# microsoft/Cream

Hardware: AMD Instinct MI355X
Metric: images/sec (whole node) AutoFormer-S supernet step @224^2 (higher is better)
Workload: dtype bf16; 1 GPU; AutoFormer-S supernet train step, random-path sampling (random.seed(epoch)), per-GPU batch 128, 224x224, AdamW, grad all-reduce RCCL; global_batch=128, parallelism=dp1, wgrad_partials=bf16 split-K partial tiles (within 1.9e-3 of fp32 partials), mixup=on-device, in the timed region

## Files before the change

### cream_amd/_lib.py

```python
import ctypes
import os

_HERE = os.path.dirname(os.path.abspath(__file__))
LIB_PATH = os.path.join(_HERE, "libcream_amd.so")

CREAM_OK = 0
_ERRORS = {
    -1: "CREAM_ERR_BAD_ARG (null pointer, negative size or unsupported stride)",
    -2: "CREAM_ERR_BAD_DTYPE (element type not supported by this entry point)",
    -3: "CREAM_ERR_LAUNCH (HIP kernel launch failed)",
    -4: "CREAM_ERR_TOO_LARGE (shape exceeds what the kernel family supports)",
}

F32, F16, BF16, F64 = 0, 1, 2, 3


class CreamLibraryError(RuntimeError):
    pass


_c = ctypes
_vp, _i, _i64, _f = _c.c_void_p, _c.c_int, _c.c_int64, _c.c_float

SIGNATURES = {
# ... 53 lines not shown
    "cream_block_wgrad_bf16": (_i, [_i]),
    "cream_colsum128_slabs": (_i, [_i]),
    "cream_colsum128": (_i, [_vp, _vp, _i, _i, _vp]),
    "cream_gelu_bwd_colsum": (_i, [_vp, _vp, _vp, _vp, _i, _i, _vp]),
    "cream_scale_cast_colsum": (_i, [_vp, _vp, _vp, _vp, _i, _i, _i, _vp]),
    "cream_grad_finalize": (_i, [_vp, _i, _vp]),
    "cream_gemm_rows_per_colsum_slab": (_i, []),
    "cream_gemm_nt256": (_i, [_i]),
    "cream_gemm_nt8": (_i, [_i]),
    "cream_linear_fwd": (_i, [_vp, _vp, _vp, _vp, _i, _i, _i, _i64, _vp]),
    "cream_linear_fwd_seg": (_i, [_vp, _vp, _vp, _vp, _i, _i, _i, _i64, _i, _i64, _vp]),
    "cream_linear_gelu_fwd": (_i, [_vp, _vp, _vp, _vp, _vp, _i, _i, _i, _i64, _vp]),
    "cream_linear_gelu_fwd_pad": (_i, [_vp, _vp, _vp, _vp, _vp, _i, _i, _i, _i, _i64, _vp]),
    "cream_linear_dgrad": (_i, [_vp, _vp, _vp, _i, _i, _i, _i64, _vp]),
    "cream_linear_dgrad_seg": (_i, [_vp, _vp, _vp, _i, _i, _i, _i64, _i, _i64, _vp]),
    "cream_linear_dgrad_mul": (_i, [_vp, _vp, _vp, _vp, _vp, _i, _i, _i, _i64, _vp]),
    "cream_linear_wgrad_splits": (_i, [_i, _i, _i]),
    "cream_linear_wgrad_splits_bf16": (_i, [_i, _i, _i]),
    "cream_gemm_tn8": (_i, [_i]),
    "cream_gemm_nthalf": (_i, [_i]),
    "cream_gemm_ntopt": (_i, [_i]),
    "cream_gemm_stagger": (_i, [_i]),
    "cream_block_layout_epoch": (_i, []),
    "cream_cu_reserve": (_i, [_i]),
    "cream_mixup_cutmix": (_i, [_vp, _vp, _vp, _i, _i, _i, _i, _i, _f, _i, _i, _i, _i, _i, _f, _vp]),
    "cream_image_batch_plan": (_i64, [_vp, _i, _i, _i]),
    "cream_image_batch_transform": (_i, [_vp, _vp, _i64, _vp, _vp, _i, _i, _i, _vp, _vp, _vp, _i64, _vp]),
    "cream_cu_count": (_i, []),
    "cream_linear_wgrad_parts": (_i, [_vp, _vp, _vp, _vp, _i, _i, _i, _i, _vp]),
    "cream_linear_wgrad_parts_bf16": (_i, [_vp, _vp, _vp, _vp, _i, _i, _i, _i, _vp]),
    "cream_param_job_tiles": (_i, [_i, _i]),
    "cream_adamw_step": (_i, [_vp, _vp, _i, _i, _i, _c.c_double, _c.c_double, _c.c_double, _c.c_double, _i64, _vp]),
    "cream_soft_ce": (_i, [_vp, _vp, _vp, _vp, _i, _i, _i, _f, _vp]),
    "cream_linear_f32_fwd": (_i, [_vp, _vp, _vp, _vp, _i, _i, _i, _i64, _i64, _i, _i, _vp]),
    "cream_bmm_f32": (_i, [_vp, _vp, _vp, _i, _i, _i, _vp, _vp, _vp, _i, _i, _vp]),
    "cream_linear_f32_dgrad": (_i, [_vp, _vp, _vp, _i, _i, _i, _i64, _i, _i, _vp]),
    "cream_linear_f32_wgrad": (_i, [_vp, _vp, _vp, _vp, _i, _i, _i, _i64, _i64, _i, _i, _vp]),
    "cream_ln_f32_fwd": (_i, [_vp, _vp, _vp, _vp, _vp, _vp, _i, _i, _f, _vp]),
    "cream_ln_f32_bwd": (_i, [_vp, _vp, _vp, _vp, _vp, _vp, _vp, _i, _i, _vp]),
    "cream_block_prof_enable": (_i, [_i]),
    "cream_block_prof_kinds": (_i, []),
    "cream_block_prof_name": (_c.c_char_p, [_i]),
    "cream_block_prof_collect": (_i, [_vp, _vp, _vp, _vp]),
    "cream_slices_copy": (_i, [_vp, _i, _vp, _i, _i, _vp]),
    "cream_block_fwd_workspace": (_i64, [_vp, _vp, _vp, _vp]),
    "cream_block_fwd": (_i, [_vp, _vp, _vp, _vp, _vp, _vp, _vp]),
    "cream_block_bwd_workspace": (_i64, [_vp, _vp, _vp, _vp]),
    "cream_block_bwd": (_i, [_vp, _vp, _vp, _vp, _vp, _vp, _vp, _vp, _i, _i64, _vp, _vp, _i, _vp, _vp]),
    "cream_image_augment_workspace": (_i64, [_i, _i, _i, _i]),
    "cream_image_augment_u8": (_i, [_vp, _vp, _i, _i, _i, _vp, _vp, _i, _vp, _i64, _vp]),
    "cream_image_batch_plan_aug": (_i64, [_vp, _i, _i, _i, _vp, _i]),
    "cream_image_batch_transform_aug": (_i, [_vp, _vp, _i64, _vp, _vp, _i, _i, _i, _vp, _vp, _vp, _vp, _i, _vp, _i64, _vp]),
}

MAX_GRAD_JOBS = 24


class GradJob(ctypes.Structure):
    _fields_ = [("dst", _vp), ("src", _vp), ("ld", _i64), ("pstride", _i64),
                ("nparts", _c.c_int32), ("rows", _c.c_int32), ("cols", _c.c_int32),
                ("interleave", _c.c_int32), ("src_bf16", _c.c_int32), ("overwrite", _c.c_int32)]

class ImageDesc(ctypes.Structure):
    _fields_ = ([("offset", _i64)] +
                [(n, _c.c_int32) for n in ("height", "width", "row_stride", "box_top", "box_left", "box_h", "box_w", "resized_h",
                                           "resized_w", "win_top", "win_left", "flip", "row0", "nrows")] +
# ... 91 lines not shown
```

### cream_amd/autoformer/block.py

```python
import ctypes
import os

import torch

from .. import _lib, timing
from . import fused_attention

def _p(t):
    return ctypes.c_void_p(t.data_ptr()) if t is not None else ctypes.c_void_p(0)


def _stream():
    return ctypes.c_void_p(torch.cuda.current_stream().cuda_stream)


def ln_fwd(x2d, gamma, beta, eps):
    M, E = x2d.shape
    y = torch.empty((M, E), dtype=torch.bfloat16, device=x2d.device)
    mean = torch.empty(M, dtype=torch.float32, device=x2d.device)
    rstd = torch.empty(M, dtype=torch.float32, device=x2d.device)
    with timing.region("ln_fwd", nbytes=M * E * 6):
        _lib.check(_lib.load().cream_ln_fwd(_p(y), _p(mean), _p(rstd), _p(x2d), _p(gamma), _p(beta), M, E,
                                           float(eps), _stream()), "cream_ln_fwd")
    return y, mean, rstd
# ... 47 lines not shown
    out = torch.empty_like(x2d)
    with timing.region("residual_add", nbytes=x2d.numel() * 10):
        _lib.check(_lib.load().cream_residual_add(_p(out), _p(x2d), _p(y), _p(sample_scale), x2d.numel(), per_sample,
                                                  _stream()), "cream_residual_add")
    return out


def scale_cast(x2d, sample_scale, per_sample):
    out = torch.empty(x2d.shape, dtype=torch.bfloat16, device=x2d.device)
    with timing.region("scale_cast", nbytes=x2d.numel() * 6):
        _lib.check(_lib.load().cream_scale_cast(_p(out), _p(x2d), _p(sample_scale), x2d.numel(), per_sample,
                                                _stream()), "cream_scale_cast")
    return out


def colsum(a):
    M, C = a.shape
    lib = _lib.load()
    partial = torch.empty((lib.cream_colsum_slabs(M), C), dtype=torch.float32, device=a.device)
    with timing.region("colsum", nbytes=a.numel() * 2):
        _lib.check(lib.cream_colsum(_p(partial), _p(a), M, C, _stream()), "cream_colsum")
    return partial.sum(dim=0)


def gelu_bwd_colsum(dg, h):
    M, C = h.shape
    lib = _lib.load()
    dh = torch.empty_like(h)
    partial = torch.empty((lib.cream_colsum128_slabs(M), C), dtype=torch.float32, device=h.device)
    with timing.region("gelu_bwd", nbytes=h.numel() * 6):
        _lib.check(lib.cream_gelu_bwd_colsum(_p(dh), _p(partial), _p(dg), _p(h), M, C, _stream()),
                   "cream_gelu_bwd_colsum")
    return dh, partial


def scale_cast_colsum(x2d, sample_scale, rows_per_sample):
    M, C = x2d.shape
    lib = _lib.load()
    out = torch.empty((M, C), dtype=torch.bfloat16, device=x2d.device)
    partial = torch.empty((lib.cream_colsum128_slabs(M), C), dtype=torch.float32, device=x2d.device)
    with timing.region("scale_cast", nbytes=x2d.numel() * 6):
        _lib.check(lib.cream_scale_cast_colsum(_p(out), _p(partial), _p(x2d), _p(sample_scale), rows_per_sample,
                                               M, C, _stream()), "cream_scale_cast_colsum")
    return out, partial


def colsum128(a):
    M, C = a.shape
    lib = _lib.load()
    partial = torch.empty((lib.cream_colsum128_slabs(M), C), dtype=torch.float32, device=a.device)
    with timing.region("colsum", nbytes=a.numel() * 2):
        _lib.check(lib.cream_colsum128(_p(partial), _p(a), M, C, _stream()), "cream_colsum128")
    return partial


def linear_fwd(x, w, bias, N, K, out=None):
    M = x.shape[0]
    if out is None:
        out = torch.empty((M, N), dtype=torch.bfloat16, device=x.device)
    with timing.region("gemm_nt", flops=2 * M * N * K):
        _lib.check(_lib.load().cream_linear_fwd(_p(out), _p(x), _p(w), _p(bias), M, N, K, w.stride(0), _stream()),
                   "cream_linear_fwd")
    return out


def linear_fwd_seg(x, w3, bias, N, K, nseg, out=None):
# ... 480 lines not shown


def head(head_mod, feat):
    return HeadFunction.apply(feat, head_mod.weight, head_mod.bias, head_mod)


class SoftTargetCEFunction(torch.autograd.Function):

    @staticmethod
    def forward(ctx, logits, target):
        lib = _lib.load()
        B, C = logits.shape
        x = logits.contiguous()
        t = target.contiguous()
        rows = torch.empty(B, dtype=torch.float32, device=x.device)
        dl = torch.empty((B, C), dtype=torch.float32, device=x.device)
        code = _lib.BF16 if x.dtype == torch.bfloat16 else _lib.F32
        _lib.check(lib.cream_soft_ce(_p(rows), _p(dl), _p(x), _p(t), B, C, code, 1.0 / B, _stream()), "cream_soft_ce")
        ctx.save_for_backward(dl)
        ctx.out_dtype = logits.dtype
        return rows.mean()

    @staticmethod
    def backward(ctx, g):
        (dl,) = ctx.saved_tensors
        out = torch.empty(dl.shape, dtype=ctx.out_dtype, device=dl.device)
        torch.mul(dl, g, out=out)
        return out, None


def soft_ce_supported(logits, target):
    return (logits.is_cuda and logits.dim() == 2 and logits.shape[1] <= 2048 and logits.dtype in (torch.bfloat16, torch.float32)
            and target.dtype == torch.float32 and target.shape == logits.shape and not target.requires_grad)


class PatchEmbedFunction(torch.autograd.Function):

    @staticmethod
    def forward(ctx, patches, weight, bias, pe, E):
        ops = patch_operands(pe)
        K = ops.w.shape[1]
        y = linear_fwd(patches, ops.w, ops.b, E, K)
        ctx.save_for_backward(patches)
        ctx.pe, ctx.E, ctx.K = pe, E, K
        return y

    @staticmethod
    def backward(ctx, dy):
        (patches,) = ctx.saved_tensors
        pe, E, K = ctx.pe, ctx.E, ctx.K
        dy = dy.to(torch.bfloat16).contiguous()
        parts, bparts = linear_wgrad_parts(dy, patches, want_bias=True)
        w = pe.proj.weight
        gw = parts.sum(0).view(E, *w.shape[1:])
        gb = bparts.sum(0)
        return None, _pad_rows(gw, w.shape[0]), _pad_rows(gb, w.shape[0]), None, None


def _pad_rows(g, rows):
    if g.shape[0] == rows:
        return g
    out = g.new_zeros((rows,) + tuple(g.shape[1:]))
    out[:g.shape[0]] = g
    return out


# ... 302 lines not shown
    ent = blk.__dict__.get(_GRADS_KEY)
    if ent is not None and all(p.grad is g for p, g in ent[1]):
        return ent[0]
    params = _block_params(blk) + (ln1.weight, ln1.bias, ln2.weight, ln2.bias) + _tables(at)
    gr = [_ensure_grad(p) for p in params]
    g = _lib.BlockGrads()
    g.wqkv, g.bqkv, g.wproj, g.bproj, g.w1, g.b1, g.w2, g.b2 = (t.data_ptr() for t in gr[:8])
    g.ld_qkv, g.ld_proj, g.ld_w1, g.ld_w2 = gr[0].stride(0), gr[2].stride(0), gr[4].stride(0), gr[6].stride(0)
    g.ln1_g, g.ln1_b, g.ln2_g, g.ln2_b = (t.data_ptr() for t in gr[8:12])
    g.tkv, g.tkh, g.tvv, g.tvh = (t.data_ptr() for t in gr[12:16])
    g.ldt = gr[12].stride(0)
    blk.__dict__[_GRADS_KEY] = (g, list(zip(params, gr)))
    return g


def _ws_layout(d):
    lib = _lib.load()
    key = (d.B, d.N, d.E, d.H, d.F, lib.cream_block_layout_epoch())
    hit = _ws_cache.get(key)
    if hit is None:
        o = [ctypes.c_int64() for _ in range(6)]
        ft = lib.cream_block_fwd_workspace(ctypes.byref(d), ctypes.byref(o[0]), ctypes.byref(o[1]), ctypes.byref(o[2]))
        bt = lib.cream_block_bwd_workspace(ctypes.byref(d), ctypes.byref(o[3]), ctypes.byref(o[4]), ctypes.byref(o[5]))
        if ft < 0 or bt < 0:
            raise RuntimeError("cream_amd: block workspace query failed")
        hit = _ws_cache[key] = (ft, o[0].value, o[1].value, o[2].value, bt, o[3].value, o[4].value, o[5].value)
    return hit


class StackFunction(torch.autograd.Function):

    @staticmethod
    def forward(ctx, x, scales, blks, *tail_args):
        tail_w, tail_b, tail_eps = (tuple(tail_args) + (None, None, 1e-5)[len(tail_args):])[:3]
        ctx.ntail = len(tail_args)
        ctx.tail = tail_w is not None
        if NATIVE_BLOCK:
            return StackFunction._forward_native(ctx, x, scales, blks, tail_w, tail_b, tail_eps)
        assert tail_w is None, "the fused tail needs the native block driver"
        B, N, E = x.shape
        M = B * N
        cur = x.contiguous().view(M, E)
        pend = None
        saved, dims = [], []
        for i, blk in enumerate(blks):
            dp1 = scales[i, 0] if scales is not None else None
            dp2 = scales[i, 1] if scales is not None else None
            x1, f, d, sv = _block_forward(blk, cur, pend, dp1, B, N)
            saved.extend(sv)
            dims.append(d)
            cur, pend = x1, (f, dp2)
        out = residual_add(cur, pend[0], pend[1], N * E)
        ctx.native = False
        ctx.blks = list(blks)
        ctx.dims = dims
        ctx.nsaved = len(saved) // len(blks)
        ctx.has_scales = scales is not None
        ctx.save_for_backward(*saved, *([scales] if scales is not None else []))
        return out.view(B, N, E)

    @staticmethod
    def _forward_native(ctx, x, scales, blks, tail_w=None, tail_b=None, tail_eps=1e-5):
        B, N, E = x.shape
        lib = _lib.load()
        x = x.contiguous()
        dev = x.device
        stream = ctypes.c_void_p(torch.cuda.current_stream(dev).cuda_stream)
        sc_ptr = scales.data_ptr() if scales is not None else 0
        cur, pend_f, pend_s = x.data_ptr(), 0, 0
        descs, wss, xptrs = [], [], []
        inference = not any(ctx.needs_input_grad)
        for i, blk in enumerate(blks):
            d = _block_desc(blk, B, N)
            d.inference = 1 if inference else 0
            ft, off_x, off_x1, off_f = _ws_layout(d)[:4]
            ws = torch.empty(ft, dtype=torch.uint8, device=dev)
            wp = ws.data_ptr()
            dp1 = sc_ptr + (2 * i) * B * 4 if sc_ptr else 0
            _lib.check(lib.cream_block_fwd(ctypes.byref(d), wp, cur, pend_f, pend_s, dp1, stream), "cream_block_fwd")
            xptrs.append(wp + off_x if pend_f else cur)
            descs.append(d)
            wss.append(ws)
            cur, pend_f, pend_s = wp + off_x1, wp + off_f, (sc_ptr + (2 * i + 1) * B * 4 if sc_ptr else 0)
        ctx.native = True
        ctx.blks = list(blks)
        ctx.descs = descs
        ctx.xptrs = xptrs
        ctx.shape = (B, N, E)
        ctx.has_scales = scales is not None
        if tail_w is not None:
            f32 = dict(dtype=torch.float32, device=dev)
            pooled, xm = torch.empty((B, E), **f32), torch.empty((B, E), **f32)
            stats = torch.empty((2, B * N), **f32)
            part = torch.empty((B, lib.cream_tail_chunks(N), E), **f32)
            gamma, beta = tail_w.detach()[:E].contiguous(), tail_b.detach()[:E].contiguous()
            _lib.check(lib.cream_tail_fwd(pooled.data_ptr(), xm.data_ptr(), part.data_ptr(), stats[0].data_ptr(),
                                          stats[1].data_ptr(), cur, pend_f, pend_s, gamma.data_ptr(), beta.data_ptr(), B, N, E,
                                          tail_eps, stream), "cream_tail_fwd")
            ctx.tail_ptrs = (cur, pend_f, pend_s)
            ctx.tail_shapes = (tuple(tail_w.shape), tuple(tail_b.shape))
            ctx.tail_params = (tail_w, tail_b) if isinstance(tail_w, torch.nn.Parameter) else None
            ctx.save_for_backward(x, *wss, *([scales] if scales is not None else []), xm, stats, gamma)
            return pooled
        out = torch.empty((B, N, E), dtype=torch.float32, device=dev)
        _lib.check(lib.cream_residual_add(out.data_ptr(), cur, pend_f, pend_s, B * N * E, N * E, stream), "cream_residual_add")
        ctx.save_for_backward(x, *wss, *([scales] if scales is not None else []))
        return out

    @staticmethod
    def backward(ctx, dout):
        if ctx.native:
            return StackFunction._backward_native(ctx, dout)
        blks = ctx.blks
        tens = ctx.saved_tensors
        scales = tens[-1] if ctx.has_scales else None
        ns = ctx.nsaved
        B, N, E = ctx.dims[0][:3]
        dx = dout.contiguous().view(B * N, E)
        L = len(blks)
        df, part = scale_cast_colsum(dx, scales[L - 1, 1] if scales is not None else None, N)
        pb2 = (part, part.shape[0], E, 0)
        for i in range(L - 1, -1, -1):
            dp1 = scales[i, 0] if scales is not None else None
            prev_scale = scales[i - 1, 1] if (scales is not None and i > 0) else None
            dx, df, pb2 = _block_backward(blks[i], ctx.dims[i], dp1, tens[i * ns:(i + 1) * ns], dx, df, pb2,
                                          prev_scale, i > 0)
        join_side_stream_at_end_of_backward(dx.device)
        return (dx.view(B, N, E), None, None) + (None, None, None)[:ctx.ntail]

    @staticmethod
    def _backward_native(ctx, dout):
        blks = ctx.blks
        tens = ctx.saved_tensors
        tail = None
        if ctx.tail:
            tens, tail = tens[:-3], tens[-3:]
        scales = tens[-1] if ctx.has_scales else None
        wss = tens[1:1 + len(blks)]
        B, N, E = ctx.shape
        M = B * N
        lib = _lib.load()
        dev = dout.device
        stream = ctypes.c_void_p(torch.cuda.current_stream(dev).cuda_stream)
        if WGRAD_SIDE_STREAM:
            side_st = _side_stream(dev)
            side = ctypes.c_void_p(side_st.cuda_stream)
        else:
            side_st, side = None, stream
        sc_ptr = scales.data_ptr() if scales is not None else 0
        L = len(blks)
        tail_grads = (None, None)
        if tail is not None:
            xm, stats, gamma = tail
            g = dout.contiguous().float()
            dx_t = torch.empty((M, E), dtype=torch.float32, device=dev)
            df_t = torch.empty((M, E), dtype=torch.bfloat16, device=dev)
            part = torch.empty((lib.cream_ln_partials(), E), dtype=torch.float32, device=dev)
            x1p, fp, sp = ctx.tail_ptrs
            _lib.check(lib.cream_tail_bwd(dx_t.data_ptr(), df_t.data_ptr(), part.data_ptr(), g.data_ptr(), x1p, fp,
                                          stats[0].data_ptr(), stats[1].data_ptr(), gamma.data_ptr(), sp, B, N, E, stream),
                       "cream_tail_bwd")
            wshape, bshape = ctx.tail_shapes
            if NATIVE_ENDS_GRADS and ctx.tail_params is not None:
                tw, tb = ctx.tail_params
                gx = g * xm
                jobs = GradJobs()
                jobs.add(tw, gx, B, E, 1, E)
                jobs.add(tb, g, B, E, 1, E)
                _accumulate_and_notify(jobs, [tw, tb])
            else:
                gw = torch.zeros(wshape, dtype=torch.float32, device=dev)
                gb = torch.zeros(bshape, dtype=torch.float32, device=dev)
                torch.sum(g * xm, dim=0, out=gw[:E])
                torch.sum(g, dim=0, out=gb[:E])
                tail_grads = (gw, gb)
        else:
            dx_t = dout.contiguous().view(M, E)
            df_t, part = scale_cast_colsum(dx_t, scales[L - 1, 1] if scales is not None else None, N)
        keep = [dx_t, df_t, part]
        dx, df, pb2, pb2_parts, pb2_stride = dx_t.data_ptr(), df_t.data_ptr(), part.data_ptr(), part.shape[0], E
        ws = None
        off_dx = 0
        for i in range(L - 1, -1, -1):
            d = ctx.descs[i]
            bt, off_dx, off_dfp, off_pl1 = _ws_layout(d)[4:]
            ws = torch.empty(bt, dtype=torch.uint8, device=dev)
            keep.append(ws)
            wp = ws.data_ptr()
            g = _block_grads(blks[i])
            dp1 = sc_ptr + (2 * i) * B * 4 if sc_ptr else 0
            prev = sc_ptr + (2 * (i - 1) + 1) * B * 4 if (sc_ptr and i > 0) else 0
            _lib.check(lib.cream_block_bwd(ctypes.byref(d), ctypes.byref(g), wss[i].data_ptr(), ctx.xptrs[i], wp, dx, df, pb2,
                                           pb2_parts, pb2_stride, dp1, prev, 1 if i > 0 else 0, stream, side),
                       "cream_block_bwd")
            if _grad_ready_hooks:
                if side_st is not None:
                    with torch.cuda.stream(side_st):
                        _notify(blks[i])
                else:
                    _notify(blks[i])
            dx, df = wp + off_dx, wp + off_dfp
            pb2, pb2_parts, pb2_stride = wp + off_pl1 + 2 * E * 4, lib.cream_ln_partials(), 3 * E
        join_side_stream_at_end_of_backward(dev, keep + [t for t in tens if t is not None and t.is_cuda])
        out = ws[off_dx:off_dx + M * E * 4].view(torch.float32).view(B, N, E)
        return (out, None, None) + (tail_grads[0], tail_grads[1], None)[:ctx.ntail]


class BlockFunction:

    @staticmethod
    def apply(x, dp1, dp2, blk):
        scales = None
        if dp1 is not None or dp2 is not None:
            ones = torch.ones(x.shape[0], device=x.device, dtype=torch.float32)
            scales = torch.stack([dp1 if dp1 is not None else ones, dp2 if dp2 is not None else ones]).unsqueeze(0)
        return StackFunction.apply(x, scales, [blk], None, None, 1e-5)
```

### cream_amd/autoformer/engine.py

```python
import random

import torch
import torch.nn.functional as F

from . import block as _block
from .supernet import Vision_TransformerSuper

SEARCH_SPACES = {
    'T': dict(embed_dim=256, depth=14, num_heads=4, mlp_ratio=4.0,
              choices=dict(mlp_ratio=[3.5, 4], num_heads=[3, 4], depth=[12, 13, 14], embed_dim=[192, 216, 240])),
    'S': dict(embed_dim=448, depth=14, num_heads=7, mlp_ratio=4.0,
              choices=dict(mlp_ratio=[3.0, 3.5, 4.0], num_heads=[5, 6, 7], depth=[12, 13, 14],
                           embed_dim=[320, 384, 448])),
    'B': dict(embed_dim=640, depth=16, num_heads=10, mlp_ratio=4.0,
              choices=dict(mlp_ratio=[3.0, 3.5, 4.0], num_heads=[8, 9, 10], depth=[14, 15, 16],
                           embed_dim=[528, 576, 624])),
}


def sample_configs(choices):
    depth = random.choice(choices['depth'])
    config = {dim: [random.choice(choices[dim]) for _ in range(depth)] for dim in ('mlp_ratio', 'num_heads')}
    config['embed_dim'] = [random.choice(choices['embed_dim'])] * depth
    config['layer_num'] = depth
    return config


def build_supernet(size='S', drop_path_rate=0.1, num_classes=1000, img_size=224, **overrides):
    s = SEARCH_SPACES[size]
    kw = dict(img_size=img_size, patch_size=16, embed_dim=s['embed_dim'], depth=s['depth'],
              num_heads=s['num_heads'], mlp_ratio=s['mlp_ratio'], qkv_bias=True, drop_rate=0.0,
              drop_path_rate=drop_path_rate, gp=True, num_classes=num_classes, max_relative_position=14,
              relative_position=True, change_qkv=True, abs_pos=True)
    kw.update(overrides)
    return Vision_TransformerSuper(**kw)


def soft_target_cross_entropy(logits, target):
    if logits.is_cuda and _block.soft_ce_supported(logits, target):
        return _block.SoftTargetCEFunction.apply(logits, target)
    return torch.sum(-target * F.log_softmax(logits.float(), dim=-1), dim=-1).mean()


def param_groups(model, weight_decay=0.05):
    skip = model.no_weight_decay() if hasattr(model, 'no_weight_decay') else set()
    decay, no_decay = [], []
    for name, p in model.named_parameters():
        if not p.requires_grad:
            continue
        (no_decay if (p.dim() <= 1 or name.endswith('.bias') or name in skip) else decay).append(p)
    return [{'params': no_decay, 'weight_decay': 0.0}, {'params': decay, 'weight_decay': weight_decay}]


class NativeAdamW(torch.optim.Optimizer):

    def __init__(self, model, param_groups, lr, betas=(0.9, 0.999), eps=1e-8):
        super().__init__(param_groups, dict(lr=lr, betas=betas, eps=eps, weight_decay=0.0))
        self.model = model
        self._cream_rewrites_operands = True
        self._steps = 0
        self._table = None
        self._grads = ()
        self._plist = ()
        self._ops = []
        for g in self.param_groups:
            for p in g['params']:
                self.state[p] = dict(exp_avg=torch.zeros_like(p, memory_format=torch.contiguous_format),
                                     exp_avg_sq=torch.zeros_like(p, memory_format=torch.contiguous_format))

    def _build(self):
        wd = {p: g['weight_decay'] for g in self.param_groups for p in g['params']}
        for p in wd:
            st = self.state[p]
            for k in ('exp_avg', 'exp_avg_sq'):
# ... 78 lines not shown
    return torch.optim.AdamW(groups, lr=scaled, betas=(0.9, 0.999), eps=1e-8)


class SupernetTrainer:

    def __init__(self, model, optimizer, choices, reducer=None, amp_dtype=torch.bfloat16, max_norm=0.0, mixup_fn=None):
        self.mixup_fn = mixup_fn
        self.model = model
        self.optimizer = optimizer
        self.choices = choices
        self.reducer = reducer
        self.amp_dtype = amp_dtype
        self.max_norm = max_norm
        self.config = None

    def start_epoch(self, epoch):
        random.seed(epoch)
        self.model.train()

    def sample(self):
        self.config = sample_configs(self.choices)
        self.model.set_sample_config(self.config)
        return self.config

    def forward_backward(self, images, target):
        dev = images.device.type
        use_amp = self.amp_dtype is not None and self.amp_dtype != torch.float32
        if self.reducer is not None:
            self.reducer.zero_grad()
            self.reducer.prepare(self.config)
        else:
            self.optimizer.zero_grad(set_to_none=False)
        with torch.autocast(device_type=dev, dtype=self.amp_dtype, enabled=use_amp):
            logits = self.model(images)
            loss = soft_target_cross_entropy(logits, target)
        loss.backward()
        if self.reducer is not None:
            self.reducer.finish()
        return loss

    def step(self, images, target):
        self.sample()
        if self.mixup_fn is not None:
            images, target = self.mixup_fn(images, target)
        loss = self.forward_backward(images, target)
        if self.max_norm and self.max_norm > 0:
            torch.nn.utils.clip_grad_norm_(self.model.parameters(), self.max_norm)
        self.optimizer.step()
        return loss


class PendingEval:

    def __init__(self, tot, n_total, config, params):
        self._tot, self._n, self._config, self._params, self._done = tot, n_total, config, params, None

    def result(self):
        if self._done is None:
            loss_sum, h1, h5 = self._tot.tolist()
            n = max(float(self._n), 1.0)
            self._done = dict(loss=loss_sum / n, acc1=100.0 * h1 / n, acc5=100.0 * h5 / n, config=self._config, params=self._params)
            self._tot = None
        return self._done


@torch.no_grad()
def evaluate(batches, model, amp_dtype=torch.bfloat16, choices=None, mode='super', retrain_config=None, defer=False):
    model.eval()
# ... 59 lines not shown
```

### cream_amd/autoformer/supernet.py

```python
import numpy as np
import os

import torch
import torch.nn as nn
import torch.nn.functional as F

from . import block as _block
from .modules import AttentionSuper, LayerNormSuper, LinearSuper, PatchembedSuper, _trunc_normal_


def _bf16_autocast(x):
    return (x.is_cuda and torch.is_autocast_enabled('cuda')
            and torch.get_autocast_dtype('cuda') == torch.bfloat16)


def gelu(x):
    return F.gelu(x.float()).type_as(x)


def calc_dropout(dropout, sample_embed_dim, super_embed_dim):
    return dropout * 1.0 * sample_embed_dim / super_embed_dim


class DropPath(nn.Module):
# ... 201 lines not shown
                                                     self.super_embed_dim))
            else:
                blk.set_sample_config(is_identity_layer=True)
        if self.pre_norm:
            self.norm.set_sample_config(self.sample_embed_dim[-1])
        self.head.set_sample_config(self.sample_embed_dim[-1], self.num_classes)

    def get_sampled_params_numel(self, config):
        self.set_sample_config(config)
        total = 0
        for name, module in self.named_modules():
            if hasattr(module, 'calc_sampled_param_num'):
                parts = name.split('.')
                if parts[0] == 'blocks' and int(parts[1]) >= config['layer_num']:
                    continue
                total += module.calc_sampled_param_num()
        return total + self.sample_embed_dim[0] * (2 + self.patch_embed_super.num_patches)

    def get_complexity(self, sequence_length):
        flops = self.patch_embed_super.get_complexity(sequence_length)
        flops += np.prod(self.pos_embed[..., :self.sample_embed_dim[0]].size()) / 2.0
        for blk in self.blocks:
            flops += blk.get_complexity(sequence_length + 1)
        flops += self.head.get_complexity(sequence_length + 1)
        return flops

    def _keep_prob(self, probs, device):
        key = (probs, str(device))
        cache = self.__dict__.setdefault('_keep_cache', {})
        if key not in cache:
            cache[key] = 1.0 - torch.tensor(probs, device=device).view(-1, 1, 1)
        return cache[key]

    def forward_features(self, x):
        B = x.shape[0]
        E = self.sample_embed_dim[0]
        if x.is_cuda and NATIVE_ENDS and _block.stem_supported(self, x):
            x = _block.stem(self, x)
        else:
            x = self.patch_embed_super(x)
            cls = self.cls_token[..., :E].expand(B, -1, -1)
            x = torch.cat((cls, x), dim=1)
            if self.abs_pos:
                x = x + self.pos_embed[..., :E]
            x = F.dropout(x, p=self.sample_dropout, training=self.training)
        active = [blk for blk in self.blocks if not blk.is_identity_layer]
        if active and _bf16_autocast(x) and all(b.fused and _block.supported(b, x) for b in active):
            scales = None
            probs = [(getattr(b.drop_path, 'drop_prob', 0.0) or 0.0) if self.training else 0.0 for b in active]
            if any(probs):
                keep = self._keep_prob(tuple(probs), x.device)
                scales = torch.floor(keep + torch.rand(len(active), 2, B, device=x.device)) / keep
            if (NATIVE_ENDS and _block.NATIVE_BLOCK and self.pre_norm and self.gp and x.shape[1] > 1
                    and self.norm.weight.dtype == torch.float32 and self.norm.bias is not None
                    and _block._no_frozen_parameters(self.norm)):
                return _block.StackFunction.apply(x, scales, active, self.norm.weight, self.norm.bias, self.norm.eps)
            x = _block.StackFunction.apply(x, scales, active, None, None, 1e-5)
        else:
            for blk in self.blocks:
                x = blk(x)
        if self.pre_norm:
            x = self.norm(x)
        if self.gp:
            return torch.mean(x[:, 1:], dim=1)
        return x[:, 0]

    def forward(self, x):
        feat = self.forward_features(x)
        if feat.is_cuda and NATIVE_ENDS and not isinstance(self.head, nn.Identity) and _block.head_supported(self.head, feat):
            return _block.head(self.head, feat)
        return self.head(feat)
```

### include/cream_amd.h

```cpp
#ifndef CREAM_AMD_H_
#define CREAM_AMD_H_

#include <stdint.h>

#ifdef __cplusplus
extern "C" {
#endif

#define CREAM_OK               0
#define CREAM_ERR_BAD_ARG     -1
#define CREAM_ERR_BAD_DTYPE   -2
#define CREAM_ERR_LAUNCH      -3
#define CREAM_ERR_TOO_LARGE   -4

#define CREAM_F32   0
#define CREAM_F16   1
#define CREAM_BF16  2
#define CREAM_F64   3

const char* cream_version(void);

const char* cream_build_info(void);


// ... 221 lines not shown
    int64_t ld;
    int64_t pstride;
    int32_t nparts, rows, cols;
    int32_t interleave;
    int32_t src_bf16;
    int32_t overwrite;
} cream_grad_job;
#define CREAM_MAX_GRAD_JOBS 24
int cream_grad_finalize(const cream_grad_job* jobs, int njobs, void* stream);

typedef struct cream_image_desc {
    int64_t offset;
    int32_t height, width, row_stride;
    int32_t box_top, box_left, box_h, box_w;
    int32_t resized_h, resized_w;
    int32_t win_top, win_left;
    int32_t flip;
    int32_t row0, nrows;
    int64_t tmp_off;
    int32_t erase_top, erase_left, erase_h, erase_w;
    uint32_t erase_seed;
    int32_t reserved;
} cream_image_desc;
int64_t cream_image_batch_plan(cream_image_desc* descs, int B, int out_h, int out_w);
int cream_image_batch_transform(float* out, const uint8_t* pixels, int64_t pixels_bytes, const cream_image_desc* descs,
                                const cream_image_desc* descs_dev, int B, int out_h, int out_w, const float* mean,
                                const float* stdev, void* workspace, int64_t workspace_bytes, void* stream);

int cream_mixup_cutmix(float* x, float* y, const int64_t* target, int B, int Cimg, int H, int W, int num_classes, float lam,
                       int use_cutmix, int yl, int yh, int xl, int xh, float label_smoothing, void* stream);

int cream_soft_ce(float* loss_rows, float* dlogits, const void* logits, const float* target, int B, int C, int logits_dtype,
                  float grad_scale, void* stream);

int cream_linear_f32_fwd(float* y, const float* x, const float* w, const float* bias, int M, int N, int K, int64_t ldx,
                         int64_t ldw, int seg, int step, void* stream);
int cream_linear_f32_dgrad(float* dx, const float* dy, const float* w, int M, int N, int K, int64_t ldw, int seg, int step,
                           void* stream);
int cream_linear_f32_wgrad(float* dw, float* dbias, const float* dy, const float* x, int M, int N, int K, int64_t ldx,
                           int64_t lddw, int seg, int step, void* stream);
int cream_bmm_f32(float* c, const float* a, const float* b, int M, int N, int K, const int64_t* a_strides,
                  const int64_t* b_strides, const int64_t* c_strides, int nb0, int nb1, void* stream);
int cream_ln_f32_fwd(float* y, float* mean, float* rstd, const float* x, const float* gamma, const float* beta,
                     int M, int E, float eps, void* stream);
int cream_ln_f32_bwd(float* dx, float* partial, const float* dy, const float* x, const float* mean, const float* rstd,
                     const float* gamma, int M, int E, void* stream);

typedef struct cream_slice_job {
    float* full;
    int64_t ld;
    int64_t packed_off;
    int32_t rows, cols;
} cream_slice_job;
int cream_slices_copy(const cream_slice_job* jobs_dev, int njobs, float* packed, int max_rows, int to_packed, void* stream);

typedef struct cream_block_desc {
    int32_t B, N, E, H, F;
    int32_t gh, gw, mr;
    int32_t F_valid, inference;
    float eps1, eps2, attn_scale;
    float reserved_f;
    const void *wqkv, *wqkv_t, *bqkv;
    const void *wproj, *wproj_t, *bproj;
    const void *w1, *w1_t, *b1;
    const void *w2, *w2_t, *b2;
    int64_t ld_qkv, ld_qkv_t, seg_qkv, seg_qkv_t, ld_proj, ld_proj_t, ld_w1, ld_w1_t, ld_w2, ld_w2_t;
// ... 74 lines not shown
```

Baseline: 14890 images/sec.

## Fuse classifier head with soft-target cross-entropy and drop-path scale computation

Adds a HIP kernel pair that fuses the final pooled LayerNorm output cast, the classifier head GEMM, the soft-target cross-entropy and its backward (dfeat, head weight/bias grads and norm gamma/beta grads) into single launches. It uses last-arrival atomic counters, and the tail norm's weight grads are deferred into the fused backward. A separate small kernel computes drop-path keep scales in one launch instead of several torch elementwise ops. The fused head path is opt-in through an environment flag and uses double-precision accumulation for the weight gradients, which may be slower than a tensor-core GEMM.

Measured after the change: 14920 images/sec (median of 6 runs). Within noise of the previous version (+0.2%).

```diff
diff --git a/cream_amd/_lib.py b/cream_amd/_lib.py
--- a/cream_amd/_lib.py
+++ b/cream_amd/_lib.py
@@ -109,6 +109,11 @@
     "cream_param_job_tiles": (_i, [_i, _i]),
     "cream_adamw_step": (_i, [_vp, _vp, _i, _i, _i, _c.c_double, _c.c_double, _c.c_double, _c.c_double, _i64, _vp]),
     "cream_soft_ce": (_i, [_vp, _vp, _vp, _vp, _i, _i, _i, _f, _vp]),
+    "cream_head_ce_supported": (_i, [_i, _i, _i]),
+    "cream_head_ce_counters": (_i, [_i]),
+    "cream_head_ce_fwd": (_i, [_vp, _vp, _vp, _vp, _vp, _vp, _vp, _i64, _vp, _vp, _i, _i, _i, _f, _vp, _vp]),
+    "cream_head_ce_bwd": (_i, [_vp, _vp, _vp, _i64, _vp, _vp, _vp, _vp, _vp, _vp, _vp, _vp, _i64, _i, _i, _i, _vp, _vp]),
+    "cream_drop_path_scales": (_i, [_vp, _vp, _vp, _i, _i, _vp]),
     "cream_linear_f32_fwd": (_i, [_vp, _vp, _vp, _vp, _i, _i, _i, _i64, _i64, _i, _i, _vp]),
     "cream_bmm_f32": (_i, [_vp, _vp, _vp, _i, _i, _i, _vp, _vp, _vp, _i, _i, _vp]),
     "cream_linear_f32_dgrad": (_i, [_vp, _vp, _vp, _i, _i, _i, _i64, _i, _i, _vp]),
diff --git a/cream_amd/autoformer/block.py b/cream_amd/autoformer/block.py
--- a/cream_amd/autoformer/block.py
+++ b/cream_amd/autoformer/block.py
@@ -103,6 +103,15 @@
         _lib.check(lib.cream_gelu_bwd_colsum(_p(dh), _p(partial), _p(dg), _p(h), M, C, _stream()),
                    "cream_gelu_bwd_colsum")
     return dh, partial
+
+
+def drop_path_scales(u, keep):
+    L = keep.numel()
+    assert u.dtype == torch.float32 and keep.dtype == torch.float32 and u.shape[0] == L and u.is_contiguous()
+    out = torch.empty_like(u)
+    _lib.check(_lib.load().cream_drop_path_scales(_p(out), _p(u), _p(keep.contiguous()), L, u.numel() // max(L, 1), _stream()),
+               "cream_drop_path_scales")
+    return out
 
 
 def scale_cast_colsum(x2d, sample_scale, rows_per_sample):
@@ -649,6 +658,83 @@
 def soft_ce_supported(logits, target):
     return (logits.is_cuda and logits.dim() == 2 and logits.shape[1] <= 2048 and logits.dtype in (torch.bfloat16, torch.float32)
             and target.dtype == torch.float32 and target.shape == logits.shape and not target.requires_grad)
+
+
+FUSED_HEAD_CE = os.environ.get('CREAM_FUSED_HEAD_CE', '0') == '1'
+_head_ce_counters = {}
+
+
+def _head_ce_counter(dev, B):
+    n = _lib.load().cream_head_ce_counters(B)
+    c = _head_ce_counters.get(dev)
+    if c is None or c.numel() < n:
+        c = _head_ce_counters[dev] = torch.zeros(max(n, 64), dtype=torch.int32, device=dev)
+    return c
+
+
+class HeadCEFunction(torch.autograd.Function):
+
+    @staticmethod
+    def forward(ctx, feat, xm, target, weight, bias, norm_w, norm_b, head):
+        lib = _lib.load()
+        ops = head_operands(head)
+        C, E = head.sample_out_dim, head.sample_in_dim
+        B = feat.shape[0]
+        dev = feat.device
+        feat = feat.contiguous()
+        t = target.contiguous()
+        x = torch.empty((B, E), dtype=torch.bfloat16, device=dev)
+        logits = torch.empty((B, C), dtype=torch.bfloat16, device=dev)
+        rows = torch.empty(B, dtype=torch.float32, device=dev)
+        loss = torch.empty((), dtype=torch.float32, device=dev)
+        dl = torch.empty((B, C), dtype=torch.float32, device=dev)
+        _lib.check(lib.cream_head_ce_fwd(_p(x), _p(logits), _p(rows), _p(loss), _p(dl), _p(feat), _p(ops.w), ops.w.stride(0),
+                                         _p(ops.b), _p(t), B, C, E, 1.0 / B, _p(_head_ce_counter(dev, B)), _stream()),
+                   "cream_head_ce_fwd")
+        ctx.save_for_backward(x, dl, xm)
+        ctx.head, ctx.dims = head, (B, C, E)
+        ctx.params = (weight, bias, norm_w, norm_b)
+        return loss
+
+    @staticmethod
+    def backward(ctx, g):
+        x, dl, xm = ctx.saved_tensors
+        lib = _lib.load()
+        B, C, E = ctx.dims
+        dev = dl.device
+        w, b, nw, nb = ctx.params
+        ops = head_operands(ctx.head, fresh=False)
+        g = g.to(torch.float32).contiguous()
+        gw, gb, gnw, gnb = (_ensure_grad(p) for p in (w, b, nw, nb))
+        dlogits = torch.empty((B, C), dtype=torch.bfloat16, device=dev)
+        dfeat = torch.empty((B, E), dtype=torch.float32, device=dev)
+        _lib.check(lib.cream_head_ce_bwd(_p(dlogits), _p(dfeat), _p(gw), gw.stride(0), _p(gb), _p(gnw), _p(gnb), _p(dl), _p(g),
+                                         _p(x), _p(xm), _p(ops.wt), ops.wt.stride(0), B, C, E, _p(_head_ce_counter(dev, B)),
+                                         _stream()), "cream_head_ce_bwd")
+        for fn in _grad_ready_hooks:
+            fn([w, b])
+            fn([nw, nb])
+        return dfeat, None, None, None, None, None, None, None
+
+
+def head_ce_supported(head, norm, B, target):
+    if not (FUSED_HEAD_CE and NATIVE_ENDS_GRADS and NATIVE_BLOCK and torch.is_grad_enabled() and target.is_cuda):
+        return False
+    if not (torch.is_autocast_enabled('cuda') and torch.get_autocast_dtype('cuda') == torch.bfloat16):
+        return False
+    if not (hasattr(head, 'sample_in_dim') and getattr(head, 'bias', None) is not None and not getattr(head, 'scale', False)
+            and head.weight.dtype == torch.float32 and head.weight.is_cuda and _no_frozen_parameters(head)):
+        return False
+    C, E = head.sample_out_dim, head.sample_in_dim
+    if not (target.dtype == torch.float32 and target.dim() == 2 and tuple(target.shape) == (B, C) and not target.requires_grad):
+        return False
+    if not (norm.weight.is_contiguous() and norm.bias is not None and norm.bias.is_contiguous()):
+        return False
+    return bool(_lib.load().cream_head_ce_supported(B, C, E))
+
+
+def head_ce(head_mod, norm, feat, xm, target):
+    return HeadCEFunction.apply(feat, xm, target, head_mod.weight, head_mod.bias, norm.weight, norm.bias, head_mod)
 
 
 class PatchEmbedFunction(torch.autograd.Function):
@@ -1017,11 +1103,11 @@
 
     @staticmethod
     def forward(ctx, x, scales, blks, *tail_args):
-        tail_w, tail_b, tail_eps = (tuple(tail_args) + (None, None, 1e-5)[len(tail_args):])[:3]
+        tail_w, tail_b, tail_eps, tail_link = (tuple(tail_args) + (None, None, 1e-5, None)[len(tail_args):])[:4]
         ctx.ntail = len(tail_args)
         ctx.tail = tail_w is not None
         if NATIVE_BLOCK:
-            return StackFunction._forward_native(ctx, x, scales, blks, tail_w, tail_b, tail_eps)
+            return StackFunction._forward_native(ctx, x, scales, blks, tail_w, tail_b, tail_eps, tail_link)
         assert tail_w is None, "the fused tail needs the native block driver"
         B, N, E = x.shape
         M = B * N
@@ -1045,7 +1131,7 @@
         return out.view(B, N, E)
 
     @staticmethod
-    def _forward_native(ctx, x, scales, blks, tail_w=None, tail_b=None, tail_eps=1e-5):
+    def _forward_native(ctx, x, scales, blks, tail_w=None, tail_b=None, tail_eps=1e-5, tail_link=None):
         B, N, E = x.shape
         lib = _lib.load()
         x = x.contiguous()
@@ -1085,6 +1171,9 @@
             ctx.tail_ptrs = (cur, pend_f, pend_s)
             ctx.tail_shapes = (tuple(tail_w.shape), tuple(tail_b.shape))
             ctx.tail_params = (tail_w, tail_b) if isinstance(tail_w, torch.nn.Parameter) else None
+            ctx.tail_deferred = tail_link is not None and NATIVE_ENDS_GRADS and ctx.tail_params is not None
+            if ctx.tail_deferred:
+                tail_link['xm'] = xm
             ctx.save_for_backward(x, *wss, *([scales] if scales is not None else []), xm, stats, gamma)
             return pooled
         out = torch.empty((B, N, E), dtype=torch.float32, device=dev)
@@ -1111,7 +1200,7 @@
             dx, df, pb2 = _block_backward(blks[i], ctx.dims[i], dp1, tens[i * ns:(i + 1) * ns], dx, df, pb2,
                                           prev_scale, i > 0)
         join_side_stream_at_end_of_backward(dx.device)
-        return (dx.view(B, N, E), None, None) + (None, None, None)[:ctx.ntail]
+        return (dx.view(B, N, E), None, None) + (None, None, None, None)[:ctx.ntail]
 
     @staticmethod
     def _backward_native(ctx, dout):
@@ -1146,7 +1235,9 @@
                                           stats[0].data_ptr(), stats[1].data_ptr(), gamma.data_ptr(), sp, B, N, E, stream),
                        "cream_tail_bwd")
             wshape, bshape = ctx.tail_shapes
-            if NATIVE_ENDS_GRADS and ctx.tail_params is not None:
+            if ctx.tail_deferred:
+                pass
+            elif NATIVE_ENDS_GRADS and ctx.tail_params is not None:
                 tw, tb = ctx.tail_params
                 gx = g * xm
                 jobs = GradJobs()
@@ -1188,7 +1279,7 @@
             pb2, pb2_parts, pb2_stride = wp + off_pl1 + 2 * E * 4, lib.cream_ln_partials(), 3 * E
         join_side_stream_at_end_of_backward(dev, keep + [t for t in tens if t is not None and t.is_cuda])
         out = ws[off_dx:off_dx + M * E * 4].view(torch.float32).view(B, N, E)
-        return (out, None, None) + (tail_grads[0], tail_grads[1], None)[:ctx.ntail]
+        return (out, None, None) + (tail_grads[0], tail_grads[1], None, None)[:ctx.ntail]
 
 
 class BlockFunction:
diff --git a/cream_amd/autoformer/engine.py b/cream_amd/autoformer/engine.py
--- a/cream_amd/autoformer/engine.py
+++ b/cream_amd/autoformer/engine.py
@@ -4,6 +4,7 @@
 import torch.nn.functional as F
 
 from . import block as _block
+from . import supernet as _supernet
 from .supernet import Vision_TransformerSuper
 
 SEARCH_SPACES = {
@@ -40,6 +41,17 @@
     if logits.is_cuda and _block.soft_ce_supported(logits, target):
         return _block.SoftTargetCEFunction.apply(logits, target)
     return torch.sum(-target * F.log_softmax(logits.float(), dim=-1), dim=-1).mean()
+
+
+def model_loss(model, images, target):
+    if (images.is_cuda and _supernet.NATIVE_ENDS and isinstance(model, Vision_TransformerSuper) and model.training
+            and model.pre_norm and _block.head_ce_supported(model.head, model.norm, images.shape[0], target)):
+        link = {}
+        feat = model.forward_features(images, tail_link=link)
+        if 'xm' in link:
+            return _block.head_ce(model.head, model.norm, feat, link['xm'], target)
+        return soft_target_cross_entropy(model.classify(feat), target)
+    return soft_target_cross_entropy(model(images), target)
 
 
 def param_groups(model, weight_decay=0.05):
@@ -184,8 +196,7 @@
         else:
             self.optimizer.zero_grad(set_to_none=False)
         with torch.autocast(device_type=dev, dtype=self.amp_dtype, enabled=use_amp):
-            logits = self.model(images)
-            loss = soft_target_cross_entropy(logits, target)
+            loss = model_loss(self.model, images, target)
         loss.backward()
         if self.reducer is not None:
             self.reducer.finish()
diff --git a/cream_amd/autoformer/supernet.py b/cream_amd/autoformer/supernet.py
--- a/cream_amd/autoformer/supernet.py
+++ b/cream_amd/autoformer/supernet.py
@@ -257,7 +257,7 @@
             cache[key] = 1.0 - torch.tensor(probs, device=device).view(-1, 1, 1)
         return cache[key]
 
-    def forward_features(self, x):
+    def forward_features(self, x, tail_link=None):
         B = x.shape[0]
         E = self.sample_embed_dim[0]
         if x.is_cuda and NATIVE_ENDS and _block.stem_supported(self, x):
@@ -275,10 +275,17 @@
             probs = [(getattr(b.drop_path, 'drop_prob', 0.0) or 0.0) if self.training else 0.0 for b in active]
             if any(probs):
                 keep = self._keep_prob(tuple(probs), x.device)
-                scales = torch.floor(keep + torch.rand(len(active), 2, B, device=x.device)) / keep
+                u = torch.rand(len(active), 2, B, device=x.device)
+                if NATIVE_ENDS and x.is_cuda:
+                    scales = _block.drop_path_scales(u, keep)
+                else:
+                    scales = torch.floor(keep + u) / keep
             if (NATIVE_ENDS and _block.NATIVE_BLOCK and self.pre_norm and self.gp and x.shape[1] > 1
                     and self.norm.weight.dtype == torch.float32 and self.norm.bias is not None
                     and _block._no_frozen_parameters(self.norm)):
+                if tail_link is not None:
+                    return _block.StackFunction.apply(x, scales, active, self.norm.weight, self.norm.bias, self.norm.eps,
+                                                      tail_link)
                 return _block.StackFunction.apply(x, scales, active, self.norm.weight, self.norm.bias, self.norm.eps)
             x = _block.StackFunction.apply(x, scales, active, None, None, 1e-5)
         else:
@@ -291,7 +298,9 @@
         return x[:, 0]
 
     def forward(self, x):
-        feat = self.forward_features(x)
+        return self.classify(self.forward_features(x))
+
+    def classify(self, feat):
         if feat.is_cuda and NATIVE_ENDS and not isinstance(self.head, nn.Identity) and _block.head_supported(self.head, feat):
             return _block.head(self.head, feat)
         return self.head(feat)
diff --git a/cream_amd/csrc/head_ce.hip b/cream_amd/csrc/head_ce.hip
--- /dev/null
+++ b/cream_amd/csrc/head_ce.hip
@@ -0,0 +1,312 @@
+#include <hip/hip_runtime.h>
+#include <stdint.h>
+
+#include "attn_common.hpp"
+#include "cream_amd.h"
+
+namespace {
+using namespace cream;
+
+constexpr int FWD_ROWS = 8;
+constexpr int CE_PER = 8;
+constexpr int KU = 16;
+
+__device__ __forceinline__ bf16x8 cvt8(const f32x4v& a, const f32x4v& b) {
+    const u32x4v v{f2bf_pair(a[0], a[1]), f2bf_pair(a[2], a[3]), f2bf_pair(b[0], b[1]), f2bf_pair(b[2], b[3])};
+    return __builtin_bit_cast(bf16x8, v);
+}
+
+__device__ __forceinline__ void nt_tile(f32x16& acc, const uint16_t* __restrict__ brow, const float* __restrict__ arow, int K,
+                                        float scale, uint16_t* keep, int g) {
+    const int steps = (K + 15) >> 4;
+    for (int ks0 = 0; ks0 < steps; ks0 += KU) {
+        bf16x8 fb[KU];
+        f32x4v lo[KU], hi[KU];
+#pragma unroll
+        for (int u = 0; u < KU; ++u) {
+            const int k = (ks0 + u) * 16;
+            const int ka = k + 8 * g < K ? k + 8 * g : 0;
+            fb[u] = *reinterpret_cast<const bf16x8*>(brow + ka);
+            lo[u] = *reinterpret_cast<const f32x4v*>(arow + ka);
+            hi[u] = *reinterpret_cast<const f32x4v*>(arow + ka + 4);
+        }
+#pragma unroll
+        for (int u = 0; u < KU; ++u) {
+            const int k = (ks0 + u) * 16;
+            if (k < K) {
+                const bool live = k + 8 * g < K;
+#pragma unroll
+                for (int i = 0; i < 4; ++i) { lo[u][i] *= scale; hi[u][i] *= scale; }
+                bf16x8 fa = cvt8(lo[u], hi[u]);
+                if (!live) { fa = bf16x8{0, 0, 0, 0, 0, 0, 0, 0}; fb[u] = fa; }
+                if (keep && live) *reinterpret_cast<bf16x8*>(keep + k + 8 * g) = fa;
+                acc = __builtin_amdgcn_mfma_f32_32x32x16_bf16(fb[u], fa, acc, 0, 0, 0);
+            }
+        }
+    }
+}
+
+__device__ __forceinline__ bool last_arrival(unsigned* counter, unsigned expected) {
+    __shared__ unsigned ticket;
+    __threadfence();
+    __syncthreads();
+    if (threadIdx.x == 0) ticket = atomicAdd(counter, 1u);
+    __syncthreads();
+    const bool last = ticket == expected - 1;
+    if (last) __threadfence();
+    return last;
+}
+
+__device__ __forceinline__ void ce_row(float* __restrict__ loss_row, float* __restrict__ d, const uint16_t* x,
+                                       const float* __restrict__ t, int C, float gscale, int lane) {
+    auto wave_red = [&](float v, bool is_max) -> float {
+#pragma unroll
+        for (int o = 32; o >= 1; o >>= 1) { const float u = __shfl_xor(v, o); v = is_max ? fmaxf(v, u) : v + u; }
+        return v;
+    };
+    float xv[4][CE_PER], tv[4][CE_PER], m4[4];
+#pragma unroll
+    for (int w = 0; w < 4; ++w)
+#pragma unroll
+        for (int i = 0; i < CE_PER; ++i) {
+            const int c = lane + 64 * w + 256 * i;
+            xv[w][i] = c < C ? bf2f((short)x[c]) : -INFINITY;
+            tv[w][i] = c < C ? t[c] : 0.f;
+        }
+#pragma unroll
+    for (int w = 0; w < 4; ++w) {
+        float mx = -INFINITY;
+#pragma unroll
+        for (int i = 0; i < CE_PER; ++i) mx = fmaxf(mx, xv[w][i]);
+        m4[w] = wave_red(mx, true);
+    }
+    const float mx = fmaxf(fmaxf(m4[0], m4[1]), fmaxf(m4[2], m4[3]));
+    float se4[4], st4[4], stx4[4];
+#pragma unroll
+    for (int w = 0; w < 4; ++w) {
+        float se = 0.f, st = 0.f, stx = 0.f;
+#pragma unroll
+        for (int i = 0; i < CE_PER; ++i) {
+            const float e = xv[w][i] == -INFINITY ? 0.f : __expf(xv[w][i] - mx);
+            se += e;
+            st += tv[w][i];
+            stx += tv[w][i] == 0.f ? 0.f : tv[w][i] * (xv[w][i] - mx);
+            xv[w][i] = e;
+        }
+        se4[w] = wave_red(se, false);
+        st4[w] = wave_red(st, false);
+        stx4[w] = wave_red(stx, false);
+    }
+    const float se = (se4[0] + se4[1]) + (se4[2] + se4[3]);
+    const float st = (st4[0] + st4[1]) + (st4[2] + st4[3]);
+    const float stx = (stx4[0] + stx4[1]) + (stx4[2] + stx4[3]);
+    const float lse = __logf(se);
+    if (lane == 0) *loss_row = st * lse - stx;
+    const float inv = 1.f / se;
+#pragma unroll
+    for (int w = 0; w < 4; ++w)
+#pragma unroll
+        for (int i = 0; i < CE_PER; ++i) {
+            const int c = lane + 64 * w + 256 * i;
+            if (c < C) d[c] = (xv[w][i] * inv * st - tv[w][i]) * gscale;
+        }
+}
+
+__global__ __launch_bounds__(256) void head_ce_fwd_kernel(uint16_t* xb, uint16_t* logits, float* loss_rows, float* loss, float* dl,
+                                                          const float* __restrict__ feat, const uint16_t* __restrict__ w,
+                                                          int64_t ldw, const uint16_t* __restrict__ bias,
+                                                          const float* __restrict__ target, int B, int C, int E, float inv_b,
+                                                          unsigned* counter) {
+    const int lane = threadIdx.x & 63, wave = threadIdx.x >> 6, c32 = lane & 31, g = lane >> 5;
+    const int m0 = blockIdx.y * FWD_ROWS, m = m0 + c32;
+    const bool mok = c32 < FWD_ROWS && m < B;
+    const int mc = min(m0 + min(c32, FWD_ROWS - 1), B - 1);
+    const int t = blockIdx.x * 4 + wave, n0 = t * 32;
+    if (n0 < C) {
+        f32x16 acc;
+#pragma unroll
+        for (int r = 0; r < 16; ++r) acc[r] = 0.f;
+        nt_tile(acc, w + (int64_t)min(n0 + c32, C - 1) * ldw, feat + (int64_t)mc * E, E, 1.f,
+                (t == 0 && mok) ? xb + (int64_t)m * E : nullptr, g);
+        if (mok) {
+#pragma unroll
+            for (int q = 0; q < 4; ++q) {
+                const int n = n0 + 8 * q + 4 * g;
+                if (n < C) {
+                    float bv[4];
+                    const u32x2v braw = *reinterpret_cast<const u32x2v*>(bias + n);
+                    bv[0] = __uint_as_float(braw[0] << 16); bv[1] = __uint_as_float(braw[0] & 0xFFFF0000u);
+                    bv[2] = __uint_as_float(braw[1] << 16); bv[3] = __uint_as_float(braw[1] & 0xFFFF0000u);
+                    *reinterpret_cast<u32x2v*>(logits + (int64_t)m * C + n) =
+                        u32x2v{f2bf_pair(acc[4 * q] + bv[0], acc[4 * q + 1] + bv[1]),
+                               f2bf_pair(acc[4 * q + 2] + bv[2], acc[4 * q + 3] + bv[3])};
+                }
+            }
+        }
+    }
+    if (!last_arrival(counter + 1 + blockIdx.y, gridDim.x)) return;
+    for (int r = wave; r < FWD_ROWS; r += 4) {
+        const int row = m0 + r;
+        if (row < B)
+            ce_row(loss_rows + row, dl + (int64_t)row * C, logits + (int64_t)row * C, target + (int64_t)row * C, C, inv_b, lane);
+    }
+    if (threadIdx.x == 0) counter[1 + blockIdx.y] = 0u;
+    if (!last_arrival(counter, gridDim.y)) return;
+    if (wave == 0) {
+        float s = 0.f;
+        for (int i = lane; i < B; i += 64) s += loss_rows[i];
+#pragma unroll
+        for (int o = 1; o <= 32; o <<= 1) s += __shfl_xor(s, o);
+        if (lane == 0) { *loss = s * inv_b; counter[0] = 0u; }
+    }
+}
+
+__global__ __launch_bounds__(64) void head_ce_bwd_kernel(uint16_t* dlogits, float* dfeat, float* gw, int64_t ldgw, float* gb,
+                                                         float* ggamma, float* gbeta, const float* __restrict__ dl,
+                                                         const float* __restrict__ gptr, const uint16_t* __restrict__ xb,
+                                                         const float* __restrict__ xm, const uint16_t* __restrict__ wt,
+                                                         int64_t ldwt, int B, int C, int E, int nA, unsigned* counter) {
+    const float gs = *gptr;
+    if ((int)blockIdx.x >= nA) {
+        const int egroups = E >> 2, idx = ((int)blockIdx.x - nA) * 64 + (int)threadIdx.x;
+        const int cg = idx / egroups, eg = idx - cg * egroups;
+        if (cg >= (C >> 2)) return;
+        const int c = 4 * cg, e = 4 * eg;
+        double acc[4][4], bacc[4];
+#pragma unroll
+        for (int i = 0; i < 4; ++i) {
+            bacc[i] = 0.0;
+#pragma unroll
+            for (int j = 0; j < 4; ++j) acc[i][j] = 0.0;
+        }
+#pragma unroll 8
+        for (int b = 0; b < B; ++b) {
+            const f32x4v d = *reinterpret_cast<const f32x4v*>(dl + (int64_t)b * C + c);
+            const u32x2v xr = *reinterpret_cast<const u32x2v*>(xb + (int64_t)b * E + e);
+            const double xv[4] = {(double)__uint_as_float(xr[0] << 16), (double)__uint_as_float(xr[0] & 0xFFFF0000u),
+                                  (double)__uint_as_float(xr[1] << 16), (double)__uint_as_float(xr[1] & 0xFFFF0000u)};
+#pragma unroll
+            for (int i = 0; i < 4; ++i) {
+                const double dv = (double)bf2f(f2bf(d[i] * gs));
+                bacc[i] += dv;
+#pragma unroll
+                for (int j = 0; j < 4; ++j) acc[i][j] = __builtin_fma(dv, xv[j], acc[i][j]);
+            }
+        }
+#pragma unroll
+        for (int i = 0; i < 4; ++i) {
+            f32x4v* dst = reinterpret_cast<f32x4v*>(gw + (int64_t)(c + i) * ldgw + e);
+            const f32x4v old = *dst;
+            *dst = f32x4v{(float)((double)old[0] + acc[i][0]), (float)((double)old[1] + acc[i][1]),
+                          (float)((double)old[2] + acc[i][2]), (float)((double)old[3] + acc[i][3])};
+            if (eg == 0) gb[c + i] = (float)((double)gb[c + i] + bacc[i]);
+        }
+        return;
+    }
+    const int lane = threadIdx.x, c32 = lane & 31, g = lane >> 5;
+    const int etiles = (E + 31) >> 5, t = (int)blockIdx.x;
+    const int mi = t / etiles, ei = t - mi * etiles, m0 = mi * 32, e0 = ei * 32, m = m0 + c32;
+    {
+        f32x16 acc;
+#pragma unroll
+        for (int r = 0; r < 16; ++r) acc[r] = 0.f;
+        nt_tile(acc, wt + (int64_t)min(e0 + c32, E - 1) * ldwt, dl + (int64_t)min(m, B - 1) * C, C, gs,
+                (ei == 0 && m < B) ? dlogits + (int64_t)m * C : nullptr, g);
+        if (m < B) {
+#pragma unroll
+            for (int q = 0; q < 4; ++q) {
+                const int e = e0 + 8 * q + 4 * g;
+                if (e < E) {
+                    f32x4v o;
+#pragma unroll
+                    for (int j = 0; j < 4; ++j) o[j] = bf2f(f2bf(acc[4 * q + j]));
+                    *reinterpret_cast<f32x4v*>(dfeat + (int64_t)m * E + e) = o;
+                }
+            }
+        }
+    }
+    if (!last_arrival(counter, (unsigned)nA)) return;
+    for (int col = lane; col < E; col += 64) {
+        double sg = 0.0, sb = 0.0;
+#pragma unroll 8
+        for (int b = 0; b < B; ++b) {
+            const double d = (double)dfeat[(int64_t)b * E + col];
+            sb += d;
+            sg = __builtin_fma(d, (double)xm[(int64_t)b * E + col], sg);
+        }
+        ggamma[col] = (float)((double)ggamma[col] + sg);
+        gbeta[col] = (float)((double)gbeta[col] + sb);
+    }
+    if (lane == 0) *counter = 0u;
+}
+
+__global__ __launch_bounds__(256) void drop_path_scales_kernel(float* __restrict__ out, const float* __restrict__ u,
+                                                               const float* __restrict__ keep, int per, int total) {
+    const int i = blockIdx.x * blockDim.x + threadIdx.x;
+    if (i >= total) return;
+    const float k = keep[i / per];
+    out[i] = floorf(k + u[i]) / k;
+}
+
+bool al16(const void* p) { return ((uintptr_t)p & 15) == 0; }
+
+}
+
+extern "C" {
+
+int cream_head_ce_supported(int B, int C, int E)
+{
+    return B > 0 && B <= (1 << 18) && C > 0 && C <= 256 * CE_PER && C % 8 == 0 && E > 0 && E % 8 == 0 && E <= (1 << 16);
+}
+
+int cream_head_ce_counters(int B) { return B <= 0 ? 0 : 1 + (B + FWD_ROWS - 1) / FWD_ROWS; }
+
+int cream_head_ce_fwd(void* x, void* logits, float* loss_rows, float* loss, float* dl, const float* feat, const void* w,
+                      int64_t ldw, const void* bias, const float* target, int B, int C, int E, float inv_b, void* counter,
+                      void* stream)
+{
+    if (B <= 0 || C <= 0 || E <= 0) return CREAM_ERR_BAD_ARG;
+    if (!cream_head_ce_supported(B, C, E)) return CREAM_ERR_TOO_LARGE;
+    if (!x || !logits || !loss_rows || !loss || !dl || !feat || !w || !bias || !target || !counter) return CREAM_ERR_BAD_ARG;
+    if (ldw < E || ldw % 8 || !al16(x) || !al16(logits) || !al16(dl) || !al16(feat) || !al16(w) || !al16(bias) ||
+        !al16(target) || ((uintptr_t)counter & 3))
+        return CREAM_ERR_BAD_ARG;
+    hipLaunchKernelGGL(head_ce_fwd_kernel, dim3((C + 127) / 128, (B + FWD_ROWS - 1) / FWD_ROWS), dim3(256), 0, (hipStream_t)stream, (uint16_t*)x,
+                       (uint16_t*)logits, loss_rows, loss, dl, feat, (const uint16_t*)w, ldw, (const uint16_t*)bias, target, B,
+                       C, E, inv_b, (unsigned*)counter);
+    return hipGetLastError() == hipSuccess ? CREAM_OK : CREAM_ERR_LAUNCH;
+}
+
+int cream_head_ce_bwd(void* dlogits, float* dfeat, float* grad_w, int64_t ld_grad_w, float* grad_b, float* grad_gamma,
+                      float* grad_beta, const float* dl, const float* g, const void* x, const float* xm, const void* wt,
+                      int64_t ldwt, int B, int C, int E, void* counter, void* stream)
+{
+    if (B <= 0 || C <= 0 || E <= 0) return CREAM_ERR_BAD_ARG;
+    if (!cream_head_ce_supported(B, C, E)) return CREAM_ERR_TOO_LARGE;
+    if (!dlogits || !dfeat || !grad_w || !grad_b || !grad_gamma || !grad_beta || !dl || !g || !x || !xm || !wt || !counter)
+        return CREAM_ERR_BAD_ARG;
+    if (ldwt < C || ldwt % 8 || ld_grad_w < E || ld_grad_w % 4 || !al16(dlogits) || !al16(dfeat) || !al16(grad_w) ||
+        !al16(dl) || !al16(x) || !al16(wt) || ((uintptr_t)counter & 3))
+        return CREAM_ERR_BAD_ARG;
+    const int nA = ((B + 31) / 32) * ((E + 31) / 32);
+    const int64_t nB = ((int64_t)(C / 4) * (E / 4) + 63) / 64;
+    if (nA + nB >= ((int64_t)1 << 31)) return CREAM_ERR_TOO_LARGE;
+    hipLaunchKernelGGL(head_ce_bwd_kernel, dim3((unsigned)(nA + nB)), dim3(64), 0, (hipStream_t)stream, (uint16_t*)dlogits, dfeat, grad_w,
+                       ld_grad_w, grad_b, grad_gamma, grad_beta, dl, g, (const uint16_t*)x, xm, (const uint16_t*)wt, ldwt, B, C,
+                       E, nA, (unsigned*)counter);
+    return hipGetLastError() == hipSuccess ? CREAM_OK : CREAM_ERR_LAUNCH;
+}
+
+int cream_drop_path_scales(float* out, const float* u, const float* keep, int L, int per, void* stream)
+{
+    if (L < 0 || per < 0) return CREAM_ERR_BAD_ARG;
+    if (L == 0 || per == 0) return CREAM_OK;
+    if (!out || !u || !keep) return CREAM_ERR_BAD_ARG;
+    if ((int64_t)L * per >= ((int64_t)1 << 31)) return CREAM_ERR_TOO_LARGE;
+    const int total = L * per;
+    hipLaunchKernelGGL(drop_path_scales_kernel, dim3((total + 255) / 256), dim3(256), 0, (hipStream_t)stream, out, u, keep, per,
+                       total);
+    return hipGetLastError() == hipSuccess ? CREAM_OK : CREAM_ERR_LAUNCH;
+}
+
+}
diff --git a/include/cream_amd.h b/include/cream_amd.h
--- a/include/cream_amd.h
+++ b/include/cream_amd.h
@@ -277,6 +277,18 @@
 
 int cream_soft_ce(float* loss_rows, float* dlogits, const void* logits, const float* target, int B, int C, int logits_dtype,
                   float grad_scale, void* stream);
+
+int cream_head_ce_supported(int B, int C, int E);
+int cream_head_ce_counters(int B);
+int cream_head_ce_fwd(void* x, void* logits, float* loss_rows, float* loss, float* dl, const float* feat, const void* w,
+                      int64_t ldw, const void* bias, const float* target, int B, int C, int E, float inv_b, void* counter,
+                      void* stream);
+
+int cream_head_ce_bwd(void* dlogits, float* dfeat, float* grad_w, int64_t ld_grad_w, float* grad_b, float* grad_gamma,
+                      float* grad_beta, const float* dl, const float* g, const void* x, const float* xm, const void* wt,
+                      int64_t ldwt, int B, int C, int E, void* counter, void* stream);
+
+int cream_drop_path_scales(float* out, const float* u, const float* keep, int L, int per, void* stream);
 
 int cream_linear_f32_fwd(float* y, const float* x, const float* w, const float* bias, int M, int N, int K, int64_t ldx,
                          int64_t ldw, int seg, int step, void* stream);
```
